# maxrmorrison/torbi

Measured on AMD Instinct MI355X. Metric: timesteps decoded/sec, 1440 states batch=512, higher is better.
Workload: dtype f32; 1 GPU; 1440 states, 500 frames, batch=512 per GPU, fp32, dense transition (BASELINE configs[2]); decode = forward + argmax + backtrace, inputs resident in HBM; parallelism=single GPU, streams=2

## Files before the change

### include/torbi_hip.h

```cpp
#ifndef TORBI_HIP_H
#define TORBI_HIP_H

#include <stddef.h>
#include <stdint.h>

#ifdef __cplusplus
extern "C" {
#endif

#define TORBI_HIP_ABI_VERSION 17

#define TORBI_HIP_OK 0
#define TORBI_HIP_EINVAL (-1)
#define TORBI_HIP_EWORKSPACE (-2)
#define TORBI_HIP_ERANGE (-3)
#define TORBI_HIP_ENODEVICE (-4)
#define TORBI_HIP_EUNSUPPORTED (-5)

int torbi_hip_abi_version(void);

const char *torbi_hip_error_string(int code);

int torbi_hip_device_count(void);

// ... 12 lines not shown
int torbi_hip_set_forward_path(int path);
int torbi_hip_forward_path(int B, int S);
int torbi_hip_forward_path_on(int B, int S, int device, unsigned flags);
int torbi_hip_last_forward_kernel(char *name_out, size_t capacity);

int torbi_hip_viterbi_decode(const float *observation, const int32_t *batch_frames,
                             const float *transition, const float *initial,
                             int32_t *indices_out, void *workspace, size_t workspace_bytes,
                             int B, int T, int S, int device, void *stream);

#define TORBI_HIP_REUSE_TRANSITION 1u
#define TORBI_HIP_COLLECT_STATS 2u
#define TORBI_HIP_SHORTEST_FIRST 256u
#define TORBI_HIP_FEW_SEEDS 512u
#define TORBI_HIP_MANY_SEEDS 1024u
int torbi_hip_viterbi_decode_ex(const float *observation, const int32_t *batch_frames,
                                const float *transition, const float *initial,
                                int32_t *indices_out, void *workspace, size_t workspace_bytes,
                                int B, int T, int S, int device, void *stream, unsigned flags);

#define TORBI_HIP_MAX_BATCHES 16
typedef struct torbi_hip_batch {
    const float *observation;
    const int32_t *batch_frames;
    int32_t *indices_out;
    void *workspace;
    size_t workspace_bytes;
    int B, T;
} torbi_hip_batch;
int torbi_hip_viterbi_decode_batches(const torbi_hip_batch *batches, int count, const float *transition,
// ... 96 lines not shown
```

### torbi_amd/_lib.py

```python
import ctypes
import os
import shutil
import subprocess

import torch

_HERE = os.path.dirname(os.path.abspath(__file__))
ROOT = os.path.dirname(_HERE)
SOURCE = os.path.join(_HERE, 'csrc', 'torbi_hip.hip')
INCLUDE = os.path.join(ROOT, 'include')
LIBRARY = os.environ.get('TORBI_HIP_LIBRARY') or os.path.join(_HERE, 'libtorbi_hip.so')
ABI_VERSION = 17

_c = ctypes
SYMBOLS = {
    'torbi_hip_abi_version': (_c.c_int, []),
    'torbi_hip_error_string': (_c.c_char_p, [_c.c_int]),
    'torbi_hip_device_count': (_c.c_int, []),
    'torbi_hip_compute_units': (_c.c_int, [_c.c_int]),
    'torbi_hip_workspace_bytes': (_c.c_size_t, [_c.c_int, _c.c_int, _c.c_int]),
    'torbi_hip_viterbi_decode': (_c.c_int, [
        _c.c_void_p, _c.c_void_p, _c.c_void_p, _c.c_void_p, _c.c_void_p,
        _c.c_void_p, _c.c_size_t, _c.c_int, _c.c_int, _c.c_int, _c.c_int, _c.c_void_p]),
    'torbi_hip_viterbi_decode_uniform': (_c.c_int, [
# ... 16 lines not shown
        _c.c_void_p, _c.c_int, _c.c_void_p, _c.c_void_p, _c.c_int, _c.c_int, _c.c_int, _c.c_int, _c.c_void_p, _c.c_uint,
        _c.POINTER(_c.c_float)]),
    'torbi_hip_band_reach_over': (_c.c_int, [_c.c_void_p, _c.c_int, _c.c_int, _c.c_void_p, _c.POINTER(_c.c_int),
                                             _c.POINTER(_c.c_int), _c.POINTER(_c.c_float)]),
    'torbi_hip_band_members_over': (_c.c_int, [_c.c_int, _c.c_int, _c.c_int, _c.c_int, _c.c_float, _c.c_int]),
    'torbi_hip_viterbi_decode_banded_over': (_c.c_int, [
        _c.c_void_p, _c.c_int, _c.c_void_p, _c.c_void_p, _c.c_int, _c.c_int, _c.c_int, _c.c_float, _c.c_int, _c.c_void_p, _c.c_uint,
        _c.POINTER(_c.c_float)]),
    'torbi_hip_preparation_bytes': (_c.c_size_t, [_c.c_int]),
    'torbi_hip_viterbi_decode_batches_prepared': (_c.c_int, [
        _c.c_void_p, _c.c_int, _c.c_void_p, _c.c_void_p, _c.c_int, _c.c_int, _c.c_void_p, _c.c_uint,
        _c.POINTER(_c.c_float), _c.c_void_p, _c.c_size_t, _c.POINTER(_c.c_int)]),
    'torbi_hip_viterbi_decode_ex': (_c.c_int, [
        _c.c_void_p, _c.c_void_p, _c.c_void_p, _c.c_void_p, _c.c_void_p,
        _c.c_void_p, _c.c_size_t, _c.c_int, _c.c_int, _c.c_int, _c.c_int, _c.c_void_p, _c.c_uint]),
    'torbi_hip_scan_stats': (_c.c_int, [_c.c_void_p, _c.c_size_t, _c.c_int, _c.c_int, _c.c_int, _c.c_void_p,
                                        _c.c_int, _c.c_void_p, _c.c_uint]),
    'torbi_hip_set_forward_path': (_c.c_int, [_c.c_int]),
    'torbi_hip_forward_path': (_c.c_int, [_c.c_int, _c.c_int]),
    'torbi_hip_forward_path_on': (_c.c_int, [_c.c_int, _c.c_int, _c.c_int, _c.c_uint]),
    'torbi_hip_last_forward_kernel': (_c.c_int, [_c.c_char_p, _c.c_size_t]),
    'torbi_hip_read_posterior': (_c.c_int, [
        _c.c_void_p, _c.c_size_t, _c.c_void_p, _c.c_void_p,
        _c.c_int, _c.c_int, _c.c_int, _c.c_int, _c.c_void_p, _c.c_uint]),
    'torbi_hip_epsilon_clamp': (_c.c_int, [_c.c_void_p, _c.c_uint64, _c.c_int, _c.c_void_p]),
    'torbi_hip_log_epsilon_clamp': (_c.c_int, [_c.c_void_p, _c.c_void_p, _c.c_uint64, _c.c_int, _c.c_void_p]),
    'torbi_hip_fill_synthetic': (_c.c_int, [
        _c.c_void_p, _c.c_uint64, _c.c_uint64, _c.c_int, _c.c_int, _c.c_int, _c.c_void_p]),
    'torbi_hip_stream_state_bytes': (_c.c_size_t, [_c.c_int, _c.c_int, _c.c_int]),
    'torbi_hip_stream_push': (_c.c_int, [
# ... 20 lines not shown
    'torbi_hip_forward_backward_band_covers': (_c.c_int, [_c.c_int, _c.c_int, _c.c_int, _c.c_int, _c.c_int, _c.c_float,
                                                         _c.c_int]),
    'torbi_hip_forward_backward_band_workspace_bytes': (_c.c_size_t, [_c.c_int, _c.c_int, _c.c_int, _c.c_int, _c.c_int]),
    'torbi_hip_forward_backward_band': (_c.c_int, [
        _c.c_void_p, _c.c_void_p, _c.c_void_p, _c.c_void_p, _c.c_int, _c.c_int, _c.c_float, _c.c_void_p, _c.c_void_p,
        _c.c_void_p, _c.c_size_t, _c.c_int, _c.c_int, _c.c_int, _c.c_int, _c.c_void_p]),
    'torbi_hip_k_best_workspace_bytes': (_c.c_size_t, [_c.c_int, _c.c_int, _c.c_int, _c.c_int]),
    'torbi_hip_k_best': (_c.c_int, [
        _c.c_void_p, _c.c_void_p, _c.c_void_p, _c.c_void_p, _c.c_void_p, _c.c_void_p, _c.c_void_p, _c.c_size_t,
        _c.c_int, _c.c_int, _c.c_int, _c.c_int, _c.c_int, _c.c_void_p]),
    'torbi_hip_k_best_uniform': (_c.c_int, [
        _c.c_void_p, _c.c_void_p, _c.c_float, _c.c_void_p, _c.c_void_p, _c.c_void_p, _c.c_void_p, _c.c_size_t,
        _c.c_int, _c.c_int, _c.c_int, _c.c_int, _c.c_int, _c.c_void_p]),
}

MAX_BATCHES = 16


class Batch(_c.Structure):
    _fields_ = [('observation', _c.c_void_p), ('batch_frames', _c.c_void_p), ('indices_out', _c.c_void_p),
                ('workspace', _c.c_void_p), ('workspace_bytes', _c.c_size_t), ('B', _c.c_int), ('T', _c.c_int)]


_LIB = None

CPU_SOURCE = os.path.join(_HERE, 'csrc', 'torbi_cpu.cpp')
CPU_LIBRARY = os.path.join(_HERE, 'libtorbi_cpu.so')
CPU_ABI_VERSION = 3
_CPU_LIB = None

# ... 27 lines not shown
    _LIB = None
    return LIBRARY


def load():
    global _LIB
    if _LIB is not None:
        return _LIB
    if not os.path.exists(LIBRARY):
        raise FileNotFoundError(
            f'{LIBRARY} is missing: the HIP extension has not been built. Run '
            '`python -c "import __graft_entry__ as g; g.build()"` (or torbi_amd._lib.build()). '
            'torbi_amd has no CPU fallback.')
    lib = ctypes.CDLL(LIBRARY)
    for name, (restype, argtypes) in SYMBOLS.items():
        fn = getattr(lib, name)
        fn.restype = restype
        fn.argtypes = argtypes
    got = lib.torbi_hip_abi_version()
    if got != ABI_VERSION:
        raise RuntimeError(f'libtorbi_hip.so ABI version {got}, expected {ABI_VERSION}: rebuild')
    _LIB = lib
    return lib


def check(code, what='torbi_hip call'):
    if code != 0:
        msg = load().torbi_hip_error_string(code)
        raise TorbiHipError(f'{what} failed with code {code}: {msg.decode() if msg else "?"}')

# ... 68 lines not shown
```

### torbi_amd/csrc/resident_forward.hpp

```cpp
#pragma once

#include <hip/hip_runtime.h>
#include <stdint.h>
#include <math.h>
#include <type_traits>

#include "pruned_forward.hpp"
#include "lazy_backtrace.hpp"
#include "nonfinite.hpp"

namespace resident {

using pruned::kBlk;
using pruned::kR;
using pruned::kTop;
using pruned::ListBlock;
using pruned::group_bcast;
using pruned::load_list_block;

constexpr int kNI = 16;
constexpr int kMaxBatches = 16;
constexpr int kRowGroup = 16;
#ifndef TORBI_TILE16_MAX_S
#define TORBI_TILE16_MAX_S pruned::kMaxS16
// ... 43 lines not shown
    unsigned *control;
    unsigned *failed;
    int R;
    unsigned long long wait_ticks;
    int spread;
};
constexpr unsigned long long kClusterWaitTicks = 25000000ull;

inline bool supported(int S) { return S >= 64 && S <= pruned::kMaxS; }

inline size_t lds_bytes(int S, int ktop = kTop) {
    const size_t S4 = ((size_t)S + 3) / 4 * 4, ni = (size_t)tile_items(S);
    return sizeof(float) * ni * S4 + sizeof(u64) * kNI * ktop + (sizeof(float) + sizeof(int)) * kNI * ktop +
           2 * sizeof(int) * kNI + 4 * sizeof(int);
}

__host__ __device__ inline int cluster_first_group(int m, int nrg, int R) { return (int)((long long)m * nrg / R); }

constexpr int kMaxOrdered = 8192;
struct OrderJob { const int32_t *frames; int32_t *order; int B, T, tile0; int32_t *hist; int32_t *route_record; int route; };
struct OrderJobs { OrderJob job[kMaxBatches]; int ascending; int n; int tiles; int32_t *tile_map; unsigned *stats;
                   unsigned *flags; int nflags;
                   int ni; };

constexpr int kOrderChunk = 2048;
__global__ __launch_bounds__(256) void order_items_kernel(OrderJobs jobs) {
    __shared__ __align__(16) int s_len[kOrderChunk];
    const OrderJob &jb = jobs.job[blockIdx.y];
    const int b = blockIdx.x * 256 + threadIdx.x;
    const int B = jb.B, T = jb.T;
// ... 154 lines not shown
#ifndef RESIDENT_EXTRA_VALU
#define RESIDENT_EXTRA_VALU 0
#endif

#ifdef RESIDENT_STAMP
constexpr int kPhases = 12;
__device__ unsigned long long g_phase[1024 * 16 * kPhases];
__device__ unsigned long long g_wgtime[1024 * 4];
#define RSTAMP(i) { const unsigned long long now_ = __builtin_readcyclecounter(); acc[i] += now_ - last; last = now_; }
#define RCOUNT(i, n) acc[i] += (n)
#else
#define RSTAMP(i)
#define RCOUNT(i, n)
#endif

template <int KW, int MAXP, bool PIPE, int KR = kR, bool CLUSTER = false, int NI = 16, bool REPAIR = false>
__global__ __launch_bounds__(64 * KW) void resident_forward_kernel(Group grp, Cluster clu, const float *__restrict__ tt,
                                                                   const float2 *__restrict__ sorted,
                                                                   const float *__restrict__ initial, int S, int SpP) {
    constexpr int kNI = NI, G = NI / 4, EPL = kBlk / G, kRowGroup = 64 / G;
    constexpr int kR = KR, kTop = KR + 1;
    static_assert(NI == 16 || NI == 8, "tiles of 16 or 8 items");
    extern __shared__ __attribute__((aligned(16))) float lds[];
    const int S4 = (S + 3) / 4 * 4;
    u64 *top = reinterpret_cast<u64 *>(lds + (size_t)kNI * S4);
    float *mtopv = reinterpret_cast<float *>(top + kNI * kTop);
    int *mtopi = reinterpret_cast<int *>(mtopv + kNI * kTop);
    int *sframes = mtopi + kNI * kTop;
    int *sitem = sframes + kNI;
    int *smisc = sitem + kNI;

    const int tid = threadIdx.x, lane = tid & 63;
    const int wave = __builtin_amdgcn_readfirstlane(tid >> 6);
    const unsigned long long clock_0 = clock64(), wall_0 = wall_clock64();
#ifdef RESIDENT_STAMP
    const unsigned long long wg_start = wall_clock64();
#endif

    int cid = blockIdx.x, member = 0;
    const int R = CLUSTER ? clu.R : 1;
    if constexpr (REPAIR) {
        if (!grp.only || grp.only[blockIdx.x] == 0u) return;
    }
    bool local = false;
    if constexpr (CLUSTER) {
// ... 44 lines not shown
    const int B = bat.B, T = bat.T;
    const int b0 = (code & 0xfffff) * kNI;
    bool odd = false;

    if (tid < kNI) {
        int f = 0;
        const int item = bat.order[b0 + tid < B ? b0 + tid : B - 1];
        if (b0 + tid < B) {
            f = bat.frames[item];
            f = f < 1 ? 1 : (f > T ? T : f);
        }
        sframes[tid] = f;
        sitem[tid] = item;
    }
    if (tid < kNI * kTop) top[tid] = 0ull;
    __syncthreads();
    int fmax = 0;
#pragma unroll
    for (int it = 0; it < kNI; ++it) fmax = max(fmax, sframes[it]);

    for (int item = 0; item < kNI; ++item) {
        const int b = sitem[item];
        const bool valid = b0 + item < B;
        const float *src = obs + (size_t)b * T * S;
        float *dst = hist + (size_t)b * T * S;
        for (int i = tid; i < S; i += 64 * KW) {
            const float v = src[i] + initial[i];
            odd = odd || nonfinite::odd(v);
            lds[i * kNI + item] = v;
            if (valid) dst[i] = v;
// ... 33 lines not shown
    ListBlock<EPL> head0, head1;
    float obnext[4] = {0.f, 0.f, 0.f, 0.f};
    if constexpr (FIXED) {
        const int rg = rg_lo + wave;
        const int jj = kRowGroup * rg + jl;
        const int jr = (rg < rg_hi && jj < S) ? jj : S - 1;
        const float2 *row = sorted + (size_t)jr * SpP + EPL * g;
        load_list_block(head0, row, 0);
        load_list_block(head1, row, kBlk);
        if (fmax > 1) {
#pragma unroll
            for (int it = 0; it < 4; ++it) obnext[it] = obs[((size_t)ib[it] * T + 1) * S + jr];
        }
    }
    unsigned stat_blocks = 0, stat_passes = 0;

    auto publish_top = [&](int row) {
        if (tid < kNI * kTop) {
            const u64 key = top[tid];
            unsigned u = (unsigned)(key >> 32);
            u ^= (u >> 31) ? 0x80000000u : 0xffffffffu;
            const float value = key ? __uint_as_float(u) : -INFINITY;
            mtopv[tid] = value;
            mtopi[tid] = key ? (0x7fffffff - (int)(unsigned)key) * S : 0;
            top[tid] = 0ull;
            const int item = tid / kTop;
            if (tid == item * kTop && member == 0 && b0 + item < B && row < sframes[item])
                bat.rowmax[(size_t)sitem[item] * T + row] = value;
        }
    };
// ... 21 lines not shown
                const float vv[4] = {v.x, v.y, v.z, v.w};
                const int oo[4] = {o.x, o.y, o.z, o.w};
#pragma unroll
                for (int r = 0; r < kR; ++r) { seedv[it][r] = vv[r]; seedo[it][r] = oo[r]; }
                thr[it] = live[it] ? vv[kR] : -INFINITY;
            } else {
#pragma unroll
                for (int r = 0; r < kR; ++r) { seedv[it][r] = mtopv[item * kTop + r]; seedo[it][r] = mtopi[item * kTop + r]; }
                thr[it] = live[it] ? mtopv[item * kTop + kR] : -INFINITY;
            }
        }
        RSTAMP(1);

        int opaque = 0;
        asm volatile("" : "+s"(opaque));
#pragma unroll
        for (int p = 0; p < MAXP; ++p) {
            const int rg = rg_lo + wave + KW * p + opaque;
            if (rg < rg_hi) {
                const int jj = kRowGroup * rg + jl;
                const bool jv = jj < S;
                const int jr = jv ? jj : S - 1;
                const float2 *row = sorted + (size_t)jr * SpP + EPL * g;
                ListBlock<EPL> cur, nxt;
                float ob[4];
                if constexpr (FIXED) {
                    cur = head0;
                    nxt = head1;
#pragma unroll
                    for (int it = 0; it < 4; ++it) ob[it] = obnext[it];
// ... 84 lines not shown
                int nblk = 1;
                consume(cur, nxt);
                load_list_block(cur, row, 2 * kBlk);
                auto fold_seeds = [&]() {
#pragma unroll
                    for (int it = 0; it < 4; ++it)
#pragma unroll
                        for (int r = 0; r < kR; ++r) best[it] = fmaxf(best[it], seedv[it][r] + seedt[it][r]);
                };
                auto more = [&](const ListBlock<EPL> &blk) {
                    if (RESIDENT_ABL & 1) return nblk < 11;
                    const float tn = group_bcast<G, 0>(blk.e[0].x);
                    return (bool)__any(jv && ((tn + thr[0] > best[0]) | (tn + thr[1] > best[1]) | (tn + thr[2] > best[2]) |
                                              (tn + thr[3] > best[3])));
                };
                const int Sp = (S + 15) / 16 * 16;
                fold_seeds();
                RSTAMP(2);
                for (int kk = kBlk; kk < Sp; kk += 2 * kBlk) {
                    if (!more(nxt)) break;
                    RCOUNT(7, 1);
                    ++nblk;
                    consume(nxt, cur);
                    load_list_block(nxt, row, kk + 2 * kBlk);
                    if (!more(cur)) break;
                    RCOUNT(7, 1);
                    ++nblk;
                    consume(cur, nxt);
                    load_list_block(cur, row, kk + 3 * kBlk);
                }
                if ((t & 15) == 1) { stat_blocks += (unsigned)nblk; stat_passes += 1u; }
                RSTAMP(3);
                u64 last4[4];
#pragma unroll
                for (int it = 0; it < 4; ++it) last4[it] = top[(4 * g + it) * kTop + kTop - 1];
#pragma unroll
                for (int it = 0; it < 4; ++it) {
#if RESIDENT_EXTRA_VALU
                    if (dummy[it] == 12345.678f) best[it] = 0.f;
#endif
                    const float o = ob[it] + best[it];
                    odd = odd || nonfinite::odd(o);
                    pend[p][it] = o;
                    if (jv && live[it] && !(RESIDENT_ABL & 8)) hist[((size_t)ib[it] * T + t) * S + jr] = o;
                    const u64 key = top_key(o, jr);
                    if (jv && key > last4[it] && !(RESIDENT_ABL & 16)) top_insert<kTop>(top + (4 * g + it) * kTop, key);
                }
                RSTAMP(4);
            }
        }
        if constexpr (CLUSTER) {
            if (t + 1 < fmax && !(RESIDENT_ABL & 128)) {
                const __amdgpu_buffer_rsrc_t xdst = buffer_of(
                    reinterpret_cast<const char *>(clu.xchg) + (size_t)(kSlots * cid + (t & (kSlots - 1))) * xbytes, xrow);
#pragma unroll
                for (int p = 0; p < MAXP; ++p) {
                    const int rg = rg_lo + wave + KW * p + opaque;
                    const int jj = kRowGroup * rg + jl;
                    if (rg < rg_hi && jj < S) {
                        const float4 row4 = make_float4(pend[p][0], pend[p][1], pend[p][2], pend[p][3]);
                        if (local) store_plain(xdst, (jj * kNI + 4 * g) * 4, row4);
                        else store_through(xdst, (jj * kNI + 4 * g) * 4, row4);
                    }
                }
            }
            RSTAMP(8);
        }
        __syncthreads();
        RSTAMP(5);
#pragma unroll
        for (int p = 0; p < MAXP; ++p) {
            const int rg = rg_lo + wave + KW * p + opaque;
            const int jj = kRowGroup * rg + jl;
            if (rg < rg_hi && jj < S)
                *reinterpret_cast<float4 *>(lds + (size_t)jj * kNI + 4 * g) =
                    make_float4(pend[p][0], pend[p][1], pend[p][2], pend[p][3]);
        }
        if constexpr (CLUSTER) {
            if (t + 1 < fmax) {
                const __amdgpu_buffer_rsrc_t xold = buffer_of(
                    reinterpret_cast<const char *>(clu.xchg) + (size_t)(kSlots * cid + ((t + 2) & (kSlots - 1))) * xbytes, xrow);
                unsigned absent_bits = kAbsentBits;
                asm volatile("" : "+v"(absent_bits));
                const float absent = __uint_as_float(absent_bits);
// ... 98 lines not shown
            }
        }
        publish_top(t);
        RSTAMP(6);
    }
    if constexpr (CLUSTER) {
        if (tid == 0 && smisc[1]) {
            atomicAdd(&grp.stats[127], 1u);
            clu.failed[cid] = 1u;
        }
    }
    if (lane == 0 && stat_passes) {
        atomicAdd(&grp.stats[0], stat_blocks);
        atomicAdd(&grp.stats[64], stat_passes);
    }
    nonfinite::raise(odd, bat.alarm, grp.serial);
    if (!REPAIR && blockIdx.x == 0 && tid == 0) {
        grp.stats[120] = (unsigned)((clock64() - clock_0) >> 4);
        grp.stats[121] = (unsigned)((wall_clock64() - wall_0) >> 4);
    }
#ifdef RESIDENT_STAMP
    if (lane == 0 && blockIdx.x < 1024)
        for (int i = 0; i < kPhases; ++i) g_phase[((size_t)blockIdx.x * 16 + wave) * kPhases + i] = acc[i];
    if (tid == 0 && blockIdx.x < 1024) {
        g_wgtime[4 * blockIdx.x] = wg_start;
        g_wgtime[4 * blockIdx.x + 1] = wall_clock64();
        g_wgtime[4 * blockIdx.x + 2] = (unsigned long long)fmax;
    }
#endif
}
// ... 50 lines not shown
```

### torbi_amd/csrc/torbi_hip.hip

```cpp

#include <hip/hip_runtime.h>
#include <algorithm>
#include <atomic>
#include <mutex>
#include <type_traits>
#include <vector>
#include <stdint.h>
#include <stddef.h>
#include <math.h>
#include <stdlib.h>

#include "torbi_hip.h"
#include "scratch.hpp"
#include "dispatch.hpp"
#include "dense_forward.hpp"
#include "lazy_backtrace.hpp"
#include "uniform_decode.hpp"
#include "pruned_forward.hpp"
#include "resident_forward.hpp"
#include "small_batch_forward.hpp"
#include "held_matrix_forward.hpp"
#include "small_states.hpp"
#include "band_forward.hpp"
#include "band_tile_forward.hpp"
// ... 414 lines not shown
               : e[0] == 'd' ? TORBI_HIP_FORWARD_DENSE
               : e[0] == 'p' ? TORBI_HIP_FORWARD_PRUNED
               : e[0] == 'r' ? TORBI_HIP_FORWARD_RESIDENT
               : e[0] == 'c' ? TORBI_HIP_FORWARD_CLUSTER
               : e[0] == 'h' ? TORBI_HIP_FORWARD_HELD
               : e[0] == 'b' ? TORBI_HIP_FORWARD_BAND : TORBI_HIP_FORWARD_AUTO;
        g_forward_path.store(v, std::memory_order_relaxed);
    }
    return v;
}
inline int requested_path(unsigned flags) {
    const unsigned f = (flags >> 4) & 7u;
    return f ? (int)f - 1 : default_path();
}
constexpr unsigned kKnownFlags = TORBI_HIP_REUSE_TRANSITION | TORBI_HIP_COLLECT_STATS | (7u << 4) | TORBI_HIP_SHORTEST_FIRST |
                                 TORBI_HIP_FEW_SEEDS | TORBI_HIP_MANY_SEEDS;
inline bool flags_ok(unsigned flags) {
    return !(flags & ~kKnownFlags) && ((flags >> 4) & 7u) <= (unsigned)TORBI_HIP_FORWARD_BAND + 1u;
}

constexpr int kMaxGroupTiles = 16384;
inline int tiles_of(int B, int S) { const int ni = resident::tile_items(S); return (B + ni - 1) / ni; }
inline bool resident_fits(int S, int tiles) { return resident::supported(S) && tiles <= kMaxGroupTiles; }

inline int cluster_members(int tiles, int S, int cus) {
    if (tiles < 1 || 2 * tiles > cus) return 1;
    int R = cus / tiles;
    const int nrg = (S + resident::pass_rows(S) - 1) / resident::pass_rows(S);
    R = std::min(R, std::min(resident::kMaxR, nrg));
    return R < 2 ? 1 : R;
}
// ... 509 lines not shown
};

inline bool few_seeds(unsigned flags, bool clusters) {
    if (flags & TORBI_HIP_FEW_SEEDS) return true;
    if (flags & TORBI_HIP_MANY_SEEDS) return false;
    return clusters;
}

template <int KW, int MAXP, int KR, bool CLUSTER, int NI, bool REPAIR = false>
hipError_t launch_resident_kernel(const resident::Group &grp, const resident::Cluster &clu, int workgroups,
                                  const ResidentWorkspace &w, const float *init, int S, hipStream_t stream) {
    const size_t lds = resident::lds_bytes(S, KR + 1);
    auto *kernel = &resident::resident_forward_kernel<KW, MAXP, true, KR, CLUSTER, NI, REPAIR>;
    const hipError_t e = ensure_dynamic_lds(kernel, lds);
    if (e != hipSuccess) return e;
    hipLaunchKernelGGL(kernel, dim3(workgroups), dim3(64 * KW), lds, stream, grp, clu, w.tt, w.sorted, init, S, w.SpP);
    if (!REPAIR)
        TORBI_NOTE_KERNEL("resident::resident_forward_kernel<%d, %d, true, %d, %s, %d, false>", KW, MAXP, KR,
                          CLUSTER ? "true" : "false", NI);
    return hipGetLastError();
}

template <int KR, int NI>
hipError_t launch_whole_tiles(const resident::Group &grp, const resident::Cluster &clu, int tiles, const ResidentWorkspace &w,
                              const float *init, int S, hipStream_t s) {
    const int nrg = (S + resident::pass_rows(S) - 1) / resident::pass_rows(S);
    if constexpr (NI != resident::kNI) {
        if (nrg <= 96) return launch_resident_kernel<12, 8, KR, false, NI>(grp, clu, tiles, w, init, S, s);
        return launch_resident_kernel<12, 11, KR, false, NI>(grp, clu, tiles, w, init, S, s);
    } else {
        if (nrg <= 72) return launch_resident_kernel<12, 6, KR, false, NI>(grp, clu, tiles, w, init, S, s);
        if (nrg <= 96) return launch_resident_kernel<12, 8, KR, false, NI>(grp, clu, tiles, w, init, S, s);
        return launch_resident_kernel<12, 11, KR, false, NI>(grp, clu, tiles, w, init, S, s);
    }
}

inline int backtrace_segments(int items) {
    const char *e = getenv("TORBI_HIP_BACKTRACE_SEGMENTS");
    const int wanted = e ? atoi(e) : 8;
    if (wanted <= 1 || items > 1024) return 1;
    return std::max(2, std::min(wanted, 2048 / std::max(items, 1)));
// ... 94 lines not shown
        const resident::OrderJob &jb = jobs.job[k];
        if (jb.B <= resident::kMaxOrdered) continue;
        const ResidentWorkspace wk = carve_resident(hb[k].workspace, hb[k].B, hb[k].T, S, cus);
        hipError_t me = hipMemsetAsync(wk.lengths_hist, 0, wk.lengths_hist_bytes, s);
        if (me != hipSuccess) return me;
        hipLaunchKernelGGL(resident::order_large_count_kernel, dim3((jb.B + 255) / 256), dim3(256), 0, s, jb);
        hipLaunchKernelGGL(resident::order_large_scan_kernel, dim3(1), dim3(1024), 0, s, jb, jobs.ascending);
        hipLaunchKernelGGL(resident::order_large_place_kernel, dim3((jb.B + 255) / 256), dim3(256), 0, s, jb);
    }
    hipLaunchKernelGGL(resident::order_tiles_kernel, dim3((tiles + 255) / 256), dim3(256), 0, s, jobs);
    return hipSuccess;
}

hipError_t run_resident(const HostBatch *hb, int n, const float *trans, const float *init, int S, int cus, hipStream_t s,
                        hipEvent_t *ev, int *launches, bool reuse, bool ascending, bool clusters, bool few,
                        Preparation *kept) {
    {
        const hipError_t ne = nonfinite_begin(hb, n, trans, init, S, s, false);
        if (ne != hipSuccess) return ne;
    }
    int tiles = 0;
    for (int k = 0; k < n; ++k) tiles += tiles_of(hb[k].B, S);
    const ResidentWorkspace w = carve_resident(hb[0].workspace, hb[0].B, hb[0].T, S, cus, kept);
    const int R = clusters ? cluster_members(tiles, S, cus) : 1;
    const int spread = (R % 8 == 0 && resident::tile_items(S) == 8) ? 1 : 0;
    resident::Cluster clu{w.xchg, w.where, tiles, w.control, w.failed, R, cluster_wait_ticks(), spread};
    if (ev) (void)hipEventRecord(ev[0], s);
    if (kept) reuse = kept->valid;
    if (!reuse) launch_list_preparation(trans, w.sorted, w.row_range, w.tt, S, w.SpP, w.NPOW, resident::tile_items(S), s);
    if (kept) kept->valid = true;
    LaunchGroup group;
    hipError_t e = assemble_group(hb, n, S, cus, s, ascending, resident::tile_items(S), R > 1 ? ROUTE_CLUSTER : ROUTE_RESIDENT,
                                  w.flags, R > 1 ? w.nflags : 0, group);
    if (e != hipSuccess) return e;
    const resident::Group &grp = group.grp;
    const int items = group.items;
    if (ev) (void)hipEventRecord(ev[3], s);
    const int nrg = (S + resident::pass_rows(S) - 1) / resident::pass_rows(S);
    const bool small = resident::tile_items(S) != resident::kNI;
    e = by_flag(few, [&](auto few_) { return by_flag(small, [&](auto small_) {
        constexpr int KR = decltype(few_)::value ? 1 : 3, NI = decltype(small_)::value ? 8 : resident::kNI;
        if (R <= 1) return launch_whole_tiles<KR, NI>(grp, clu, tiles, w, init, S, s);
        {
            const size_t granules = (size_t)tiles * resident::kSlots * resident::cluster_slot_bytes(S) / 16;
            hipLaunchKernelGGL(resident::absent_kernel, dim3((unsigned)std::min<size_t>((granules + 255) / 256, 2048)), dim3(256),
                               0, s, reinterpret_cast<uint4 *>(w.xchg), granules);
        }
        const int passes = ((nrg + R - 1) / R + 11) / 12;
        const int grid = 8 * ((tiles + 7) / 8) * R;
        const int share = (nrg + R - 1) / R;
        hipError_t ce;
        if constexpr (NI == 8) {
            if (share <= 8) ce = launch_resident_kernel<8, 1, KR, true, NI>(grp, clu, grid, w, init, S, s);
            else if (share <= 16) ce = launch_resident_kernel<8, 2, KR, true, NI>(grp, clu, grid, w, init, S, s);
            else if (passes <= 2) ce = launch_resident_kernel<12, 2, KR, true, NI>(grp, clu, grid, w, init, S, s);
            else if (passes <= 4) ce = launch_resident_kernel<12, 4, KR, true, NI>(grp, clu, grid, w, init, S, s);
            else ce = launch_resident_kernel<12, 6, KR, true, NI>(grp, clu, grid, w, init, S, s);
// ... 192 lines not shown
    const float *const obs = hb.obs;
    const int32_t *const frames = hb.frames;
    int32_t *const out = hb.out;
    void *const workspace = hb.workspace;
    const int B = hb.B, T = hb.T;
    hipError_t e;
    const int cus = cu_count(device);
    Route route = route_for(path, B, S, cus);
    if (route == ROUTE_HELD && path == TORBI_HIP_FORWARD_AUTO && other_streams_busy(device, s))
        route = route_for(path, B, S, cus, false);
    if (route == ROUTE_HELD && !held_resident(S, device, cus))
        route = route_for(path == TORBI_HIP_FORWARD_HELD ? TORBI_HIP_FORWARD_AUTO : path, B, S, cus, false);
    if (taken) *taken = route;
    if (route == ROUTE_RESIDENT || route == ROUTE_CLUSTER)
        return run_resident(&hb, 1, trans, init, S, cus, s, ev, launches, reuse, false, route == ROUTE_CLUSTER,
                            few_seeds(seed_flags, route == ROUTE_CLUSTER), kept);
    if (kept) reuse = false;
    if (ev) (void)hipEventRecord(ev[0], s);
    if (ev) (void)hipEventRecord(ev[3], s);
    e = nonfinite_begin(&hb, 1, trans, init, S, s, route != ROUTE_SMALL, -1, -1, route != ROUTE_SMALL);
    if (e != hipSuccess) return e;
    if (route == ROUTE_SMALL) {
        const Workspace w = carve(workspace, B, T, S);
        e = small::supported(S) ? launch_small(obs, frames, trans, init, w, out, hb.record, B, T, S, s, launches, cus)
                                : launch_block(obs, frames, trans, init, w, out, hb.record, B, T, S, s, launches, cus);
        if (ev) (void)hipEventRecord(ev[1], s);
        if (e == hipSuccess) e = nonfinite_end(&hb, 1, trans, init, S, s);
        if (ev) (void)hipEventRecord(ev[2], s);
        return e;
    }
    e = stamp_route(hb.record, route, s);
// ... 122 lines not shown
    const bool together = resident_fits(S, tiles) &&
                          (path == TORBI_HIP_FORWARD_RESIDENT || path == TORBI_HIP_FORWARD_CLUSTER ||
                           (path == TORBI_HIP_FORWARD_AUTO && !small::supported(S) && !small_block_auto((int)std::min(items, 1ll << 30), S, cus) &&
                            (2 * tiles > cus || (split && largest > 16))));
    const bool clusters = together && split && path != TORBI_HIP_FORWARD_RESIDENT;
    const bool ascending = (flags & TORBI_HIP_SHORTEST_FIRST) != 0;
    PhaseEvents pe(phase_ms != nullptr);
    if (pe.err != hipSuccess) return (int)pe.err;
    int launches = 0, covered = n;
    Route taken = ROUTE_BAND;
    hipError_t e = hipSuccess;
    if (banded) {
        e = run_band(hb, n, transition, initial, S, band_choice, cus, s, pe.events(), &launches, ascending);
    } else if (together) {
        e = run_resident(hb, n, transition, initial, S, cus, s, pe.events(), &launches, reuse, ascending, clusters,
                         few_seeds(flags, clusters), call.preparation);
        taken = clusters ? ROUTE_CLUSTER : ROUTE_RESIDENT;
    } else {
        for (int k = 0; k < n && e == hipSuccess; ++k)
            e = run_decode(hb[k], transition, initial, S, device, s, k == n - 1 ? pe.events() : nullptr, &launches,
                           reuse && k == 0, path, flags, &taken, call.preparation);
        covered = 1;
    }
    mark_decode_end(device, s);
    if (phase_ms) {
        if (e == hipSuccess) e = pe.read(phase_ms);
        phase_ms[2] = (float)launches;
        phase_ms[3] = (float)taken;
        phase_ms[5] = (float)covered;
    }
    return (int)e;
}

}

extern "C" {

int torbi_hip_abi_version(void) { return TORBI_HIP_ABI_VERSION; }

const char *torbi_hip_error_string(int code) {
    switch (code) {
        case TORBI_HIP_OK: return "success";
        case TORBI_HIP_EINVAL: return "invalid argument (null pointer, non-positive dimension or unknown flag)";
        case TORBI_HIP_EWORKSPACE: return "workspace smaller than torbi_hip_workspace_bytes()";
        case TORBI_HIP_ERANGE: return "problem dimensions out of range for this build";
        case TORBI_HIP_ENODEVICE: return "no usable HIP device";
        case TORBI_HIP_EUNSUPPORTED: return "shape not covered by this specialised entry point";
        default: break;
    }
    if (code > 0) return hipGetErrorString(static_cast<hipError_t>(code));
    return "unknown torbi_hip error";
}

// ... 715 lines not shown
```

### torbi_amd/viterbi.py

```python
import threading
import ctypes
import os
import weakref
from typing import Optional

import torch

from . import _lib, inputs, state
from .state import _version_of


def _require_gpu():
    if not torch.cuda.is_available():
        raise RuntimeError(
            'torbi_amd.decode needs a HIP device (PyTorch-ROCm reports none). This package has '
            'no CPU fallback (decode_cpu is the CPU operator); the reference CPU implementation is only restated under '
            'oracle/ as a test oracle.')


def _check_inputs(observation, batch_frames, transition, initial):
    shape = inputs.check_shapes(observation, batch_frames, transition, initial)
    for name, tensor, dtype in (('observation', observation, torch.float32),
                                ('transition', transition, torch.float32),
                                ('initial', initial, torch.float32),
# ... 95 lines not shown
                if known[4] >= known[2]:
                    known[4] = 0
                    known[2] = min(2 * known[2], DENSE_PROBE_AT_MOST)
                    return False
    return losing


FEW_SEEDS_GATE = 0.17


def _seed_flag(transition: torch.Tensor, states: int) -> int:
    depth = _known_depth(transition, states)
    if depth is None:
        return 0
    return 512 if depth <= FEW_SEEDS_GATE * states / 16.0 else 1024


def _seeds_kept(flags: int, chosen: str, tiles: int, device) -> int:
    if flags & 512:
        return 1
    if flags & 1024:
        return 3
    return 1 if chosen != 'resident' and 2 * tiles <= compute_units(device) else 3


def _few_seeds(transition: torch.Tensor, states: int) -> bool:
    return _seed_flag(transition, states) == 512


def _watch_resident(transition, workspace, batch, frames, states, seeds=3) -> None:
# ... 207 lines not shown
            largest = B
        if first is None and B > 0:
            first = k
        items += B
        tiles += tiles_of(B, S)
    first = first or 0
    chosen, band = _resolve(trans, transition, largest, S, device, path, tiles, count, items)
    flags = _path_flag(chosen)
    if _reusable(workspaces[first], transition, holds + (chosen, stream.value), reuse_preparation) \
            and (chosen in TIME_RESIDENT or count == 1):
        flags |= 1
    if shortest_first:
        flags |= 256
    if chosen in TIME_RESIDENT:
        flags |= _seed_flag(transition, S)
    phases = (ctypes.c_float * 6)() if _profile is not None else None
    kept = _kept_preparation(transition, largest, S, chosen, device, index) if own_scratch and chosen != 'band' else None
    model = (trans.data_ptr(), init.data_ptr(), S)
    if count == 1 and band is None and kept is None and phases is None and not shortest_first:
        (B, T, _), ws = shapes[0], workspaces[0]
        _lib.check(lib.torbi_hip_viterbi_decode_ex(observations[0].data_ptr(), batch_frames[0].data_ptr(), model[0], model[1],
                                                   indices[0].data_ptr(), ws.data_ptr(), ws.numel(), B, T, S, index, stream,
                                                   flags), 'torbi_hip_viterbi_decode_ex')
    else:
        table = (_lib.Batch * count)(*(
            _lib.Batch(obs.data_ptr(), frames.data_ptr(), found.data_ptr(), ws.data_ptr(), ws.numel(), B, T)
            for obs, frames, found, ws, (B, T, _) in zip(observations, batch_frames, indices, workspaces, shapes)))
        if band is not None:
            left, right, background = band
            _lib.check(lib.torbi_hip_viterbi_decode_banded_over(table, count, *model, left, right, ctypes.c_float(background),
# ... 239 lines not shown
```

Baseline: 57.89 million timesteps/s.

## Cap per-row sorted-list scan and defer long tails to a shared LDS queue

Adds a capped variant of the resident forward kernel. Once a row's pruned scan over its sorted transition list reaches a block-count cap, the remaining open items go into an LDS queue instead of continuing. After the pass, all waves finish those queued rows cooperatively, so a few long scans no longer hold up the whole workgroup. The cap comes from a host rule based on measured seed depth and applies only on the few-seeds path. This adds atomics, LDS usage, an extra sync and a second tail loop, and may trigger rarely or cost more than it saves when scans are short.

```diff
diff --git a/include/torbi_hip.h b/include/torbi_hip.h
--- a/include/torbi_hip.h
+++ b/include/torbi_hip.h
@@ -50,6 +50,8 @@
 #define TORBI_HIP_SHORTEST_FIRST 256u
 #define TORBI_HIP_FEW_SEEDS 512u
 #define TORBI_HIP_MANY_SEEDS 1024u
+#define TORBI_HIP_SCAN_CAP(blocks) (((unsigned)(blocks) & 127u) << 24)
+int torbi_hip_scan_cap_rule(float blocks_per_pass, int S);
 int torbi_hip_viterbi_decode_ex(const float *observation, const int32_t *batch_frames,
                                 const float *transition, const float *initial,
                                 int32_t *indices_out, void *workspace, size_t workspace_bytes,
diff --git a/torbi_amd/_lib.py b/torbi_amd/_lib.py
--- a/torbi_amd/_lib.py
+++ b/torbi_amd/_lib.py
@@ -54,6 +54,7 @@
     'torbi_hip_viterbi_decode_ex': (_c.c_int, [
         _c.c_void_p, _c.c_void_p, _c.c_void_p, _c.c_void_p, _c.c_void_p,
         _c.c_void_p, _c.c_size_t, _c.c_int, _c.c_int, _c.c_int, _c.c_int, _c.c_void_p, _c.c_uint]),
+    'torbi_hip_scan_cap_rule': (_c.c_int, [_c.c_float, _c.c_int]),
     'torbi_hip_scan_stats': (_c.c_int, [_c.c_void_p, _c.c_size_t, _c.c_int, _c.c_int, _c.c_int, _c.c_void_p,
                                         _c.c_int, _c.c_void_p, _c.c_uint]),
     'torbi_hip_set_forward_path': (_c.c_int, [_c.c_int]),
@@ -104,6 +105,8 @@
         _c.c_int, _c.c_int, _c.c_int, _c.c_int, _c.c_int, _c.c_void_p]),
 }
 
+OPTIONAL = ('torbi_hip_scan_cap_rule',)
+
 MAX_BATCHES = 16
 
 
@@ -161,6 +164,9 @@
             'torbi_amd has no CPU fallback.')
     lib = ctypes.CDLL(LIBRARY)
     for name, (restype, argtypes) in SYMBOLS.items():
+        if name in OPTIONAL and not hasattr(lib, name):
+            setattr(lib, name, None)
+            continue
         fn = getattr(lib, name)
         fn.restype = restype
         fn.argtypes = argtypes
diff --git a/torbi_amd/csrc/resident_forward.hpp b/torbi_amd/csrc/resident_forward.hpp
--- a/torbi_amd/csrc/resident_forward.hpp
+++ b/torbi_amd/csrc/resident_forward.hpp
@@ -81,6 +81,14 @@
     return sizeof(float) * ni * S4 + sizeof(u64) * kNI * ktop + (sizeof(float) + sizeof(int)) * kNI * ktop +
            2 * sizeof(int) * kNI + 4 * sizeof(int);
 }
+
+constexpr int kTailQueueMax = 3072, kTailQueueMin = 512;
+inline int tail_queue_records(int S, int ktop = kTop) {
+    const size_t fixed = lds_bytes(S, ktop) + 4 * sizeof(unsigned), all = 160 * 1024;
+    const size_t fit = fixed < all ? (all - fixed) / sizeof(uint2) : 0;
+    return (int)(fit < (size_t)kTailQueueMax ? fit : (size_t)kTailQueueMax);
+}
+inline size_t tail_queue_bytes(int records) { return 4 * sizeof(unsigned) + sizeof(uint2) * (size_t)records; }
 
 __host__ __device__ inline int cluster_first_group(int m, int nrg, int R) { return (int)((long long)m * nrg / R); }
 
@@ -265,13 +273,16 @@
 #define RCOUNT(i, n)
 #endif
 
-template <int KW, int MAXP, bool PIPE, int KR = kR, bool CLUSTER = false, int NI = 16, bool REPAIR = false>
+template <int KW, int MAXP, bool PIPE, int KRX = kR, bool CLUSTER = false, int NI = 16, bool REPAIR = false>
 __global__ __launch_bounds__(64 * KW) void resident_forward_kernel(Group grp, Cluster clu, const float *__restrict__ tt,
                                                                    const float2 *__restrict__ sorted,
-                                                                   const float *__restrict__ initial, int S, int SpP) {
+                                                                   const float *__restrict__ initial, int S, int SpP, int cap, int qcap) {
+    constexpr bool TAIL = KRX < 0;
+    constexpr int KR = TAIL ? -KRX : KRX;
     constexpr int kNI = NI, G = NI / 4, EPL = kBlk / G, kRowGroup = 64 / G;
     constexpr int kR = KR, kTop = KR + 1;
     static_assert(NI == 16 || NI == 8, "tiles of 16 or 8 items");
+    static_assert(!TAIL || (NI == 16 && !CLUSTER && !REPAIR && 4 * MAXP <= 32), "the capped scan: whole 16-item tiles, 8 passes");
     extern __shared__ __attribute__((aligned(16))) float lds[];
     const int S4 = (S + 3) / 4 * 4;
     u64 *top = reinterpret_cast<u64 *>(lds + (size_t)kNI * S4);
@@ -280,6 +291,8 @@
     int *sframes = mtopi + kNI * kTop;
     int *sitem = sframes + kNI;
     int *smisc = sitem + kNI;
+    unsigned *qhdr = reinterpret_cast<unsigned *>(smisc + 4);
+    uint2 *queue = reinterpret_cast<uint2 *>(qhdr + 4);
 
     const int tid = threadIdx.x, lane = tid & 63;
     const int wave = __builtin_amdgcn_readfirstlane(tid >> 6);
@@ -354,6 +367,7 @@
         sitem[tid] = item;
     }
     if (tid < kNI * kTop) top[tid] = 0ull;
+    if (TAIL && tid < 4) qhdr[tid] = 0u;
     __syncthreads();
     int fmax = 0;
 #pragma unroll
@@ -417,6 +431,7 @@
         }
     }
     unsigned stat_blocks = 0, stat_passes = 0;
+    unsigned stat_deferred = 0, stat_finish = 0;
 
     auto publish_top = [&](int row) {
         if (tid < kNI * kTop) {
@@ -468,6 +483,12 @@
 
         int opaque = 0;
         asm volatile("" : "+s"(opaque));
+        const int capt = (TAIL && cap > 0 && (t & 15) != 1) ? cap : 0x7fffffff;
+        unsigned *const hdr = qhdr + 2 * (t & 1);
+        unsigned dmask = 0u;
+        int qbase[MAXP];
+#pragma unroll
+        for (int p = 0; p < MAXP; ++p) qbase[p] = -1;
 #pragma unroll
         for (int p = 0; p < MAXP; ++p) {
             const int rg = rg_lo + wave + KW * p + opaque;
@@ -582,16 +603,52 @@
                     return (bool)__any(jv && ((tn + thr[0] > best[0]) | (tn + thr[1] > best[1]) | (tn + thr[2] > best[2]) |
                                               (tn + thr[3] > best[3])));
                 };
+                auto defer = [&](const ListBlock<EPL> &blk) {
+                    const float tn = group_bcast<G, 0>(blk.e[0].x);
+                    bool open[4];
+                    u64 bal[4];
+                    int total = 0;
+#pragma unroll
+                    for (int it = 0; it < 4; ++it) {
+                        open[it] = jv && (tn + thr[it] > best[it]);
+                        bal[it] = __ballot(open[it]);
+                        total += __popcll(bal[it]);
+                    }
+                    int base = 0;
+                    if (lane == 0) base = (int)atomicAdd(hdr, (unsigned)total);
+                    base = __builtin_amdgcn_readfirstlane(base);
+                    if (base + total > qcap) {
+                        if (base <= qcap && lane == 0) hdr[1] = (unsigned)base;
+                        return false;
+                    }
+                    qbase[p] = base;
+                    stat_deferred += (unsigned)total;
+#pragma unroll
+                    for (int it = 0; it < 4; ++it) {
+                        const int at = base + (int)__builtin_amdgcn_mbcnt_hi((unsigned)(bal[it] >> 32),
+                                                                             __builtin_amdgcn_mbcnt_lo((unsigned)bal[it], 0u));
+                        if (open[it]) {
+                            queue[at] = make_uint2((unsigned)jr | (unsigned)(4 * g + it) << 16, __float_as_uint(best[it]));
+                            dmask |= 1u << (4 * p + it);
+                        }
+                        base += __popcll(bal[it]);
+                    }
+                    return true;
+                };
                 const int Sp = (S + 15) / 16 * 16;
                 fold_seeds();
                 RSTAMP(2);
                 for (int kk = kBlk; kk < Sp; kk += 2 * kBlk) {
                     if (!more(nxt)) break;
+                    if constexpr (TAIL)
+                        if (nblk == capt && defer(nxt)) break;
                     RCOUNT(7, 1);
                     ++nblk;
                     consume(nxt, cur);
                     load_list_block(nxt, row, kk + 2 * kBlk);
                     if (!more(cur)) break;
+                    if constexpr (TAIL)
+                        if (nblk == capt && defer(cur)) break;
                     RCOUNT(7, 1);
                     ++nblk;
                     consume(cur, nxt);
@@ -608,11 +665,12 @@
                     if (dummy[it] == 12345.678f) best[it] = 0.f;
 #endif
                     const float o = ob[it] + best[it];
-                    odd = odd || nonfinite::odd(o);
+                    const bool mine = !TAIL || !(dmask >> (4 * p + it) & 1u);
+                    odd = odd || (mine && nonfinite::odd(o));
                     pend[p][it] = o;
-                    if (jv && live[it] && !(RESIDENT_ABL & 8)) hist[((size_t)ib[it] * T + t) * S + jr] = o;
+                    if (mine && jv && live[it] && !(RESIDENT_ABL & 8)) hist[((size_t)ib[it] * T + t) * S + jr] = o;
                     const u64 key = top_key(o, jr);
-                    if (jv && key > last4[it] && !(RESIDENT_ABL & 16)) top_insert<kTop>(top + (4 * g + it) * kTop, key);
+                    if (mine && jv && key > last4[it] && !(RESIDENT_ABL & 16)) top_insert<kTop>(top + (4 * g + it) * kTop, key);
                 }
                 RSTAMP(4);
             }
@@ -636,6 +694,74 @@
         }
         __syncthreads();
         RSTAMP(5);
+        if constexpr (TAIL) {
+            const unsigned tail = hdr[0];
+            const int nrec = __builtin_amdgcn_readfirstlane((int)(tail <= (unsigned)qcap ? tail : hdr[1]));
+            if (tid < 2) qhdr[2 * ((t + 1) & 1) + tid] = 0u;
+            if (nrec > 0) {
+                const int Sp = (S + 15) / 16 * 16;
+                const int share = (nrec + KW - 1) / KW;
+                const int r_end = min(nrec, (wave + 1) * share);
+                for (int r0 = wave * share; r0 < r_end; r0 += 64) {
+                    const int r = r0 + lane;
+                    const bool act = r < r_end;
+                    const uint2 rec = queue[act ? r : r0];
+                    const int jr = (int)(rec.x & 0xffffu), item = (int)(rec.x >> 16);
+                    float best = __uint_as_float(rec.y);
+                    const float thr = act ? mtopv[item * kTop + kR] : -INFINITY;
+                    const int b = sitem[item];
+                    const size_t cell = ((size_t)b * T + t) * S + jr;
+                    const float ob = obs[cell];
+                    const float2 *row = sorted + (size_t)jr * SpP;
+                    const char *pcol = reinterpret_cast<const char *>(lds) + 4 * item;
+                    float4 cur[kBlk / 2], nxt[kBlk / 2];
+                    int k = capt;
+#pragma unroll
+                    for (int h = 0; h < kBlk / 2; ++h) cur[h] = *reinterpret_cast<const float4 *>(row + k * kBlk + 2 * h);
+                    for (; k * kBlk < Sp; ++k) {
+                        const bool walk = cur[0].x + thr > best;
+                        if (!__any(walk)) break;
+#pragma unroll
+                        for (int h = 0; h < kBlk / 2; ++h)
+                            nxt[h] = *reinterpret_cast<const float4 *>(row + (k + 1) * kBlk + 2 * h);
+                        stat_finish += 1u;
+                        if (walk) {
+#pragma unroll
+                            for (int h = 0; h < kBlk / 2; ++h) {
+                                const float p0 = *reinterpret_cast<const float *>(pcol + __float_as_int(cur[h].y));
+                                const float p1 = *reinterpret_cast<const float *>(pcol + __float_as_int(cur[h].w));
+                                best = fmaxf(fmaxf(best, cur[h].x + p0), cur[h].z + p1);
+                            }
+                        }
+#pragma unroll
+                        for (int h = 0; h < kBlk / 2; ++h) cur[h] = nxt[h];
+                    }
+                    if (act) {
+                        const float o = ob + best;
+                        odd = odd || nonfinite::odd(o);
+                        hist[cell] = o;
+                        top_insert<kTop>(top + item * kTop, top_key(o, jr));
+                        queue[r].y = __float_as_uint(o);
+                    }
+                }
+                __syncthreads();
+#pragma unroll
+                for (int p = 0; p < MAXP; ++p) {
+                    if (qbase[p] >= 0) {
+                        int at = qbase[p];
+#pragma unroll
+                        for (int it = 0; it < 4; ++it) {
+                            const bool d = dmask >> (4 * p + it) & 1u;
+                            const u64 bal = __ballot(d);
+                            const int slot = at + (int)__builtin_amdgcn_mbcnt_hi((unsigned)(bal >> 32),
+                                                                                 __builtin_amdgcn_mbcnt_lo((unsigned)bal, 0u));
+                            if (d) pend[p][it] = __uint_as_float(queue[slot].y);
+                            at += __popcll(bal);
+                        }
+                    }
+                }
+            }
+        }
 #pragma unroll
         for (int p = 0; p < MAXP; ++p) {
             const int rg = rg_lo + wave + KW * p + opaque;
@@ -764,6 +890,10 @@
         atomicAdd(&grp.stats[0], stat_blocks);
         atomicAdd(&grp.stats[64], stat_passes);
     }
+    if (TAIL && lane == 0 && stat_deferred) {
+        atomicAdd(&grp.stats[124], stat_deferred);
+        atomicAdd(&grp.stats[125], stat_finish);
+    }
     nonfinite::raise(odd, bat.alarm, grp.serial);
     if (!REPAIR && blockIdx.x == 0 && tid == 0) {
         grp.stats[120] = (unsigned)((clock64() - clock_0) >> 4);
diff --git a/torbi_amd/csrc/torbi_hip.hip b/torbi_amd/csrc/torbi_hip.hip
--- a/torbi_amd/csrc/torbi_hip.hip
+++ b/torbi_amd/csrc/torbi_hip.hip
@@ -452,7 +452,7 @@
     return f ? (int)f - 1 : default_path();
 }
 constexpr unsigned kKnownFlags = TORBI_HIP_REUSE_TRANSITION | TORBI_HIP_COLLECT_STATS | (7u << 4) | TORBI_HIP_SHORTEST_FIRST |
-                                 TORBI_HIP_FEW_SEEDS | TORBI_HIP_MANY_SEEDS;
+                                 TORBI_HIP_FEW_SEEDS | TORBI_HIP_MANY_SEEDS | TORBI_HIP_SCAN_CAP(127);
 inline bool flags_ok(unsigned flags) {
     return !(flags & ~kKnownFlags) && ((flags >> 4) & 7u) <= (unsigned)TORBI_HIP_FORWARD_BAND + 1u;
 }
@@ -992,17 +992,46 @@
     auto *kernel = &resident::resident_forward_kernel<KW, MAXP, true, KR, CLUSTER, NI, REPAIR>;
     const hipError_t e = ensure_dynamic_lds(kernel, lds);
     if (e != hipSuccess) return e;
-    hipLaunchKernelGGL(kernel, dim3(workgroups), dim3(64 * KW), lds, stream, grp, clu, w.tt, w.sorted, init, S, w.SpP);
+    hipLaunchKernelGGL(kernel, dim3(workgroups), dim3(64 * KW), lds, stream, grp, clu, w.tt, w.sorted, init, S, w.SpP, 0, 0);
     if (!REPAIR)
         TORBI_NOTE_KERNEL("resident::resident_forward_kernel<%d, %d, true, %d, %s, %d, false>", KW, MAXP, KR,
                           CLUSTER ? "true" : "false", NI);
     return hipGetLastError();
 }
 
+template <int MAXP>
+hipError_t launch_capped_kernel(const resident::Group &grp, const resident::Cluster &clu, int workgroups,
+                                const ResidentWorkspace &w, const float *init, int S, int cap, int records, hipStream_t stream) {
+    const size_t lds = resident::lds_bytes(S, 2) + resident::tail_queue_bytes(records);
+    auto *kernel = &resident::resident_forward_kernel<12, MAXP, true, -1, false, resident::kNI, false>;
+    const hipError_t e = ensure_dynamic_lds(kernel, lds);
+    if (e != hipSuccess) return e;
+    hipLaunchKernelGGL(kernel, dim3(workgroups), dim3(64 * 12), lds, stream, grp, clu, w.tt, w.sorted, init, S, w.SpP, cap, records);
+    TORBI_NOTE_KERNEL("resident::resident_forward_kernel<12, %d, true, -1, false, 16, false>", MAXP);
+    return hipGetLastError();
+}
+
+inline const char *scan_cap_override() { return getenv("TORBI_HIP_SCAN_CAP"); }
+struct ScanCap { int cap, records; };
+inline ScanCap scan_cap_for(int cap, int S, bool few, bool whole_tiles) {
+    if (const char *e = scan_cap_override()) cap = atoi(e);
+    const int nrg = (S + resident::pass_rows(S) - 1) / resident::pass_rows(S);
+    int records = resident::tail_queue_records(S, 2);
+    if (cap < 1 || !few || !whole_tiles || resident::tile_items(S) != resident::kNI || nrg > 96 ||
+        records < resident::kTailQueueMin)
+        return ScanCap{0, 0};
+    if (const char *q = getenv("TORBI_HIP_SCAN_QUEUE")) records = std::max(1, std::min(records, atoi(q)));
+    return ScanCap{std::min(cap, 127), records};
+}
+
 template <int KR, int NI>
 hipError_t launch_whole_tiles(const resident::Group &grp, const resident::Cluster &clu, int tiles, const ResidentWorkspace &w,
-                              const float *init, int S, hipStream_t s) {
+                              const float *init, int S, hipStream_t s, ScanCap capped) {
     const int nrg = (S + resident::pass_rows(S) - 1) / resident::pass_rows(S);
+    if constexpr (KR == 1 && NI == resident::kNI) {
+        if (capped.cap > 0 && nrg <= 72) return launch_capped_kernel<6>(grp, clu, tiles, w, init, S, capped.cap, capped.records, s);
+        if (capped.cap > 0 && nrg <= 96) return launch_capped_kernel<8>(grp, clu, tiles, w, init, S, capped.cap, capped.records, s);
+    }
     if constexpr (NI != resident::kNI) {
         if (nrg <= 96) return launch_resident_kernel<12, 8, KR, false, NI>(grp, clu, tiles, w, init, S, s);
         return launch_resident_kernel<12, 11, KR, false, NI>(grp, clu, tiles, w, init, S, s);
@@ -1127,7 +1156,7 @@
 
 hipError_t run_resident(const HostBatch *hb, int n, const float *trans, const float *init, int S, int cus, hipStream_t s,
                         hipEvent_t *ev, int *launches, bool reuse, bool ascending, bool clusters, bool few,
-                        Preparation *kept) {
+                        Preparation *kept, int cap = 0) {
     {
         const hipError_t ne = nonfinite_begin(hb, n, trans, init, S, s, false);
         if (ne != hipSuccess) return ne;
@@ -1151,9 +1180,11 @@
     if (ev) (void)hipEventRecord(ev[3], s);
     const int nrg = (S + resident::pass_rows(S) - 1) / resident::pass_rows(S);
     const bool small = resident::tile_items(S) != resident::kNI;
+    if (R <= 1 && !small && scan_cap_override() && atoi(scan_cap_override()) > 0) few = true;
+    const ScanCap capped = scan_cap_for(cap, S, few, R <= 1);
     e = by_flag(few, [&](auto few_) { return by_flag(small, [&](auto small_) {
         constexpr int KR = decltype(few_)::value ? 1 : 3, NI = decltype(small_)::value ? 8 : resident::kNI;
-        if (R <= 1) return launch_whole_tiles<KR, NI>(grp, clu, tiles, w, init, S, s);
+        if (R <= 1) return launch_whole_tiles<KR, NI>(grp, clu, tiles, w, init, S, s, capped);
         {
             const size_t granules = (size_t)tiles * resident::kSlots * resident::cluster_slot_bytes(S) / 16;
             hipLaunchKernelGGL(resident::absent_kernel, dim3((unsigned)std::min<size_t>((granules + 255) / 256, 2048)), dim3(256),
@@ -1376,7 +1407,7 @@
     if (taken) *taken = route;
     if (route == ROUTE_RESIDENT || route == ROUTE_CLUSTER)
         return run_resident(&hb, 1, trans, init, S, cus, s, ev, launches, reuse, false, route == ROUTE_CLUSTER,
-                            few_seeds(seed_flags, route == ROUTE_CLUSTER), kept);
+                            few_seeds(seed_flags, route == ROUTE_CLUSTER), kept, (int)((seed_flags >> 24) & 127u));
     if (kept) reuse = false;
     if (ev) (void)hipEventRecord(ev[0], s);
     if (ev) (void)hipEventRecord(ev[3], s);
@@ -1529,7 +1560,7 @@
         e = run_band(hb, n, transition, initial, S, band_choice, cus, s, pe.events(), &launches, ascending);
     } else if (together) {
         e = run_resident(hb, n, transition, initial, S, cus, s, pe.events(), &launches, reuse, ascending, clusters,
-                         few_seeds(flags, clusters), call.preparation);
+                         few_seeds(flags, clusters), call.preparation, (int)((flags >> 24) & 127u));
         taken = clusters ? ROUTE_CLUSTER : ROUTE_RESIDENT;
     } else {
         for (int k = 0; k < n && e == hipSuccess; ++k)
@@ -1552,6 +1583,12 @@
 extern "C" {
 
 int torbi_hip_abi_version(void) { return TORBI_HIP_ABI_VERSION; }
+
+int torbi_hip_scan_cap_rule(float blocks_per_pass, int S) {
+    const float row_blocks = (float)((S + 15) / 16);
+    if (!(blocks_per_pass >= 6.0f) || 20.0f * blocks_per_pass > 13.0f * row_blocks) return 0;
+    return std::min(127, std::max(4, (int)(3.0f * blocks_per_pass / 4.0f)));
+}
 
 const char *torbi_hip_error_string(int code) {
     switch (code) {
diff --git a/torbi_amd/viterbi.py b/torbi_amd/viterbi.py
--- a/torbi_amd/viterbi.py
+++ b/torbi_amd/viterbi.py
@@ -133,6 +133,14 @@
     if depth is None:
         return 0
     return 512 if depth <= FEW_SEEDS_GATE * states / 16.0 else 1024
+
+
+def _cap_flag(transition: torch.Tensor, states: int, flags: int) -> int:
+    rule = _lib.load().torbi_hip_scan_cap_rule
+    depth = _known_depth(transition, states)
+    if rule is None or depth is None or not flags & 512:
+        return 0
+    return (int(rule(depth * ONE_SEED_DEPTH, states)) & 127) << 24
 
 
 def _seeds_kept(flags: int, chosen: str, tiles: int, device) -> int:
@@ -370,6 +378,7 @@
         flags |= 256
     if chosen in TIME_RESIDENT:
         flags |= _seed_flag(transition, S)
+        flags |= _cap_flag(transition, S, flags)
     phases = (ctypes.c_float * 6)() if _profile is not None else None
     kept = _kept_preparation(transition, largest, S, chosen, device, index) if own_scratch and chosen != 'band' else None
     model = (trans.data_ptr(), init.data_ptr(), S)
```

New measurement: 55.21 million timesteps/s. 0.954x the previous value.
